# mmigas/LiverRenderer

Hardware: AMD Instinct MI355X
Metric: Msamples/s (higher is better)
Workload: dtype f32; 1 GPU; C3 Liver-SingleMesh volpath 1920x1080 512 spp max_depth 12 (homogeneous medium, isotropic phase, envmap); width=1920, height=1080, spp=512, parallelism=1 GPU

## Files before the change

### liverrenderer_amd/csrc/film.h

```cpp

template <typename FP> DEV float estrin10(float x, FP c) {
    float x2 = x * x, x4 = x2 * x2, x8 = x4 * x4;
    float a0 = fma_(x, c[1], c[0]), a1 = fma_(x, c[3], c[2]), a2 = fma_(x, c[5], c[4]), a3 = fma_(x, c[7], c[6]), a4 = fma_(x, c[9], c[8]);
    float b0 = fma_(x2, a1, a0), b1 = fma_(x2, a3, a2);
    float c0 = fma_(x4, b1, b0);
    return fma_(x8, a4, c0);
}
DEV float rfilter_eval(FilmRef F, float x) {
    if (F.rfilter == LRT_RFILTER_GAUSSIAN) return fmax_(estrin10(sqr(x), F.rf_coeff), 0.f);
    if (F.rfilter == LRT_RFILTER_TENT) return fmax_(0.f, 1.f - __builtin_fabsf(x * F.rf_inv_radius));
    return (x >= -0.5f && x < 0.5f) ? 1.f : 0.f;
}

DEV size_t film_pixel_index(FilmRef F, int px, int py) {
    return (size_t) (py - F.crop_offset_y) * F.width + (px - F.crop_offset_x);
}

struct FilmFootprint {
    int pix, piy; float relx, rely;
    DEV uint32_t key() const { return (uint32_t) (piy + 0x4000) << 16 | (uint32_t) (pix + 0x4000); }
};
DEV FilmFootprint film_footprint(FilmRef F, int px, int py, float jx, float jy) {
    const float spx = (float) px + jx, spy = (float) py + jy;
    FilmFootprint f;
    f.pix = (int) __builtin_floorf(spx) - F.fn; f.piy = (int) __builtin_floorf(spy) - F.fn;
    f.relx = (float) f.pix + .5f - spx; f.rely = (float) f.piy + .5f - spy;
    return f;
}

DEV void finish_path(SceneRef sc, RpRef rp, float *__restrict__ film, float *__restrict__ sample_out,
                     uint64_t sample_base, uint32_t lane, V3 L, bool valid) {
    if (rp.integrator == LRT_INTEGRATOR_PATH && !valid) L = V3(0.f);
    if (sample_out) {
        const uint64_t j = lane_local_index(rp, lane);
        float4 *o = reinterpret_cast<float4 *>(sample_out) + (j - sample_base);
        *o = make_float4(L.x, L.y, L.z, valid ? 1.f : 0.f);
        return;
    }
    FilmRef F = sc.film;
    int px, py; lane_to_pixel(sc, rp, lane, &px, &py);
    const int C = F.channels;
    const float alpha = valid ? 1.f : 0.f;
    auto splat = [&](float *p, float w) {
        atomicAdd(p + 0, L.x * w); atomicAdd(p + 1, L.y * w); atomicAdd(p + 2, L.z * w);
        if (F.has_alpha) { atomicAdd(p + 3, alpha * w); atomicAdd(p + 4, 1.f * w); } else atomicAdd(p + 3, 1.f * w);
    };
    if (F.rfilter == LRT_RFILTER_BOX) {
        int x = px - F.crop_offset_x, y = py - F.crop_offset_y;
        float *p = film + ((size_t) y * F.width + x) * C;
        atomicAdd(p + 0, L.x); atomicAdd(p + 1, L.y); atomicAdd(p + 2, L.z);
        if (F.has_alpha) { atomicAdd(p + 3, alpha); atomicAdd(p + 4, 1.f); } else atomicAdd(p + 3, 1.f);
        return;
    }
    float jx, jy; lane_jitter(rp, lane, lane_local_index(rp, lane), jx, jy);
    const FilmFootprint fp = film_footprint(F, px, py, jx, jy);
    int count = F.fcount;
    for (int ys = 0; ys < count; ++ys) {
        int y = fp.piy - F.crop_offset_y + ys;
        float wy = rfilter_eval(F, fp.rely + (float) ys);
        if (y < 0 || y >= F.height || (wy == 0.f && finite3(L))) continue;
        for (int xs = 0; xs < count; ++xs) {
            int x = fp.pix - F.crop_offset_x + xs;
            if (x < 0 || x >= F.width) continue;
            float w = wy * rfilter_eval(F, fp.relx + (float) xs);
            if (w == 0.f && finite3(L)) continue;
            splat(film + ((size_t) y * F.width + x) * C, w);
        }
    }
}

struct FilmRun { uint32_t pixel; bool head, tail; };
DEV FilmRun film_run(FilmRef F, bool have, int px, int py) {
    FilmRun r;
    r.pixel = have ? (uint32_t) film_pixel_index(F, px, py) : 0xffffffffu;
    const uint32_t prev = wave_prev(r.pixel, 0xfffffffeu), next = wave_next(r.pixel, 0xfffffffeu);
    r.head = r.pixel != prev || !have; r.tail = have && r.pixel != next;
    return r;
}

DEV void finish_paths_wave(SceneRef sc, RpRef rp, float *__restrict__ film, float *__restrict__ sample_out,
                           uint64_t sample_base, bool finishing, uint32_t lane, V3 L, bool valid) {
    FilmRef F = sc.film;
    if (sample_out || F.rfilter != LRT_RFILTER_BOX) {
        if (finishing) finish_path(sc, rp, film, sample_out, sample_base, lane, L, valid);
        return;
    }
    if (rp.integrator == LRT_INTEGRATOR_PATH && !valid) L = V3(0.f);
    uint32_t pixel = 0xffffffffu;
    if (finishing) { int px, py; lane_to_pixel(sc, rp, lane, &px, &py); pixel = (uint32_t) (py - F.crop_offset_y) * (uint32_t) F.width + (uint32_t) (px - F.crop_offset_x); }
    if (__ballot(finishing) == 0ull) return;
    const uint32_t prev = wave_prev(pixel, 0xfffffffeu), next = wave_next(pixel, 0xfffffffeu);
    float v[5] = { finishing ? L.x : 0.f, finishing ? L.y : 0.f, finishing ? L.z : 0.f, finishing ? 1.f : 0.f, (finishing && valid) ? 1.f : 0.f };
    wave_segmented_sums(v, pixel != prev || !finishing);
    if (finishing && pixel != next) {
        float *p = film + (size_t) pixel * F.channels;
        atomicAdd(p + 0, v[0]); atomicAdd(p + 1, v[1]); atomicAdd(p + 2, v[2]);
        if (F.has_alpha) { atomicAdd(p + 3, v[4]); atomicAdd(p + 4, v[3]); } else atomicAdd(p + 3, v[3]);
    }
}

template <int NC, int WI, typename Live, typename Flush>
DEV void film_walk(FilmRef F, bool have, const FilmFootprint &fp, const float (&v)[NC], Live live, Flush flush) {
    const uint32_t me = threadIdx.x & 63u, key = fp.key();
    const int count = F.fcount, n_cells = count * count;
    unsigned long long todo = __ballot(have);
    while (todo) {
        const int leader = __ffsll((long long) todo) - 1;
        const bool mine = have && key == (uint32_t) __shfl((int) key, leader);
        const int gx = __shfl(fp.pix, leader), gy = __shfl(fp.piy, leader);
        float t[NC];
#pragma unroll
        for (int k = 0; k < NC; ++k) t[k] = 0.f;
        for (int ys = 0, ci = 0; ys < count; ++ys) {
            const float wy = mine ? rfilter_eval(F, fp.rely + (float) ys) : 0.f;
            for (int xs = 0; xs < count; ++xs, ++ci) {
                const float w = mine ? wy * rfilter_eval(F, fp.relx + (float) xs) : 0.f;
                const bool keep = (int) me == (ci & 63);
#pragma unroll
                for (int k = 0; k < NC; ++k) {
                    if (!live(k)) continue;
                    const float s = wave_sum(mine ? v[k] * w : 0.f);
                    if (keep) t[k] = s;
                }
                if ((ci & 63) != 63 && ci != n_cells - 1) continue;
                const int cell = (ci & ~63) + (int) me;
                bool add = false;
#pragma unroll
                for (int k = 0; k < NC; ++k) add = add || ((WI < 0 || k == WI) ? t[k] != 0.f : t[k] != t[k]);
                if (cell <= ci && add) {
                    const int cy = cell / count, cx = cell - cy * count;
                    const int x = gx - F.crop_offset_x + cx, y = gy - F.crop_offset_y + cy;
                    if (x >= 0 && x < F.width && y >= 0 && y < F.height) flush(x, y, t);
                }
#pragma unroll
                for (int k = 0; k < NC; ++k) t[k] = 0.f;
            }
        }
        todo &= ~__ballot(mine);
    }
}
```

### liverrenderer_amd/csrc/kernels.h

```cpp
#pragma once
#include "dshade.h"
#include "record.h"

namespace lrt {

#ifndef LRT_STAMP_KIND
#define LRT_STAMP_KIND 0
#endif
struct StampClock {
    unsigned long long *acc; unsigned long long t; bool on;
    DEV void start(unsigned long long *a, bool enable) { acc = a; on = enable; t = on ? __builtin_amdgcn_s_memtime() : 0ull; }
    DEV void at(int k) { if (on) { const unsigned long long now = __builtin_amdgcn_s_memtime(); if ((threadIdx.x & 63u) == 0) atomicAdd(&acc[k], now - t); t = now; } }
};

template <bool LD>
DEV uint64_t lane_rng_inc(RpRef rp, uint32_t lane) {
    if (LD) {
        const uint32_t pixel = (rp.log2_spp != 0xffffffffu) ? (lane >> rp.log2_spp) : (lane / rp.spp);
        uint32_t v0, v1; tea32(rp.base_seed, rp.spp * pixel + rp.seed, &v0, &v1);
        return (uint64_t) v0 | ((uint64_t) (rp.pass_index * rp.spp + (lane - pixel * rp.spp)) << 32);
    }
    uint32_t v0, v1; tea32(rp.seed_value, lane, &v0, &v1);
    return ((uint64_t) v1 << 1) | 1u;
}
template <bool LD>
DEV SamplerT<LD> lane_rng_fresh(RpRef rp, uint32_t lane) {
    SamplerT<LD> r; r.ld_count = rp.ld_count;
    if (LD) { r.state = 0; r.inc = lane_rng_inc<LD>(rp, lane); r.ld_prepare(); return r; }
    uint32_t v0, v1; tea32(rp.seed_value, lane, &v0, &v1);
    r.seed(v0, v1); return r;
}
template <bool LD>
DEV SamplerT<LD> lane_rng_resume(RpRef rp, uint32_t lane, uint64_t state) {
    SamplerT<LD> r; r.ld_count = rp.ld_count; r.state = state; r.inc = lane_rng_inc<LD>(rp, lane); r.ld_prepare(); return r;
}
template <bool LD>
DEV SamplerT<LD> lane_rng_resume_word(RpRef rp, uint32_t lane, uint64_t state, uint32_t word) {
    SamplerT<LD> r; r.ld_count = rp.ld_count; r.state = state;
    if (LD) {
        const uint32_t pixel = (rp.log2_spp != 0xffffffffu) ? (lane >> rp.log2_spp) : (lane / rp.spp);
        r.inc = (uint64_t) word | ((uint64_t) (rp.pass_index * rp.spp + (lane - pixel * rp.spp)) << 32);
    } else r.inc = ((uint64_t) word << 1) | 1u;
    r.ld_prepare(); return r;
}
template <bool LD> DEV uint32_t lane_rng_word(const SamplerT<LD> &r) { return LD ? (uint32_t) r.inc : (uint32_t) (r.inc >> 1); }
DEV uint64_t lane_local_index(RpRef rp, uint32_t lane) {
    if (!rp.pixel_slot) return lane;
    const uint32_t pixel = (rp.log2_spp != 0xffffffffu) ? (lane >> rp.log2_spp) : (lane / rp.spp);
    return (uint64_t) rp.pixel_slot[pixel] * rp.spp + (lane - pixel * rp.spp);
}
DEV uint32_t slot_to_lane(RpRef rp, const uint32_t *__restrict__ pixel_list, uint64_t j) {
    if (!pixel_list) return (uint32_t) j;
    const uint32_t pj = (rp.log2_spp != 0xffffffffu) ? (uint32_t) (j >> rp.log2_spp) : (uint32_t) (j / rp.spp);
    return pixel_list[pj] * rp.spp + (uint32_t) (j - (uint64_t) pj * rp.spp);
}
template <bool LD>
DEV SamplerT<LD> lane_rng_pass_start(RpRef rp, uint32_t lane, uint64_t j) {
    SamplerT<LD> r = lane_rng_fresh<LD>(rp, lane);
    if (!LD && rp.pass_index > 0) r.state = rp.pass_in[j];
    return r;
}
DEV void lane_jitter(RpRef rp, uint32_t lane, uint64_t j, float &jx, float &jy) {
    if (rp.ld_count) { SamplerT<true> r = lane_rng_pass_start<true>(rp, lane, j); r.next2(jx, jy); }
    else { SamplerT<false> r = lane_rng_pass_start<false>(rp, lane, j); r.next2(jx, jy); }
}

DEV void lane_to_pixel(SceneRef sc, RpRef rp, uint32_t lane, int *px, int *py) {
    uint32_t idx = (rp.log2_spp != 0xffffffffu) ? (lane >> rp.log2_spp) : (lane / rp.spp);
    uint32_t W = (uint32_t) sc.film.width;
    uint32_t y = idx / W, x = idx - y * W;
    *px = (int) x + sc.film.crop_offset_x; *py = (int) y + sc.film.crop_offset_y;
}

DEV Ray camera_ray(SceneRef sc, float ax, float ay) {
    const LRT_CONST float *m = sc.cam.s2c;
    V3 p(ax + sc.cam.ppo_x, ay + sc.cam.ppo_y, 0.f);
    float r[4];
#pragma unroll
    for (int i = 0; i < 4; ++i) r[i] = fma_(m[4 * i + 2], p.z, fma_(m[4 * i + 1], p.y, fma_(m[4 * i + 0], p.x, m[4 * i + 3])));
    V3 near_p(r[0] / r[3], r[1] / r[3], r[2] / r[3]);
    V3 d = normalize(near_p);
    Ray ray;
    ray.o = V3(sc.cam.to_world[3], sc.cam.to_world[7], sc.cam.to_world[11]);
    ray.d = xform_vec12(sc.cam.to_world, d);
    float inv_z = rcp(d.z), near_t = sc.cam.near_clip * inv_z, far_t = sc.cam.far_clip * inv_z;
    ray.o = ray.o + ray.d * near_t;
    ray.maxt = far_t - near_t;
    return ray;
}

template <bool LD, bool ENTRY = false>
DEV PathState generate_camera_path(SceneRef sc, RpRef rp, const uint32_t *__restrict__ pixel_list, uint64_t j, uint32_t *entry = nullptr) {
    uint32_t lane;
    if (pixel_list) { uint32_t pj = (rp.log2_spp != 0xffffffffu) ? (uint32_t) (j >> rp.log2_spp) : (uint32_t) (j / rp.spp); lane = pixel_list[pj] * rp.spp + (uint32_t) (j - (uint64_t) pj * rp.spp); }
    else lane = (uint32_t) j;
    if (ENTRY && sc.primary_enabled) *entry = sc.primary_tab[(rp.log2_spp != 0xffffffffu) ? (lane >> rp.log2_spp) : (lane / rp.spp)];
    SamplerT<LD> rng = lane_rng_pass_start<LD>(rp, lane, j);
    int px, py; lane_to_pixel(sc, rp, lane, &px, &py);
    float jx, jy; rng.next2(jx, jy);
    float spx = (float) px + jx, spy = (float) py + jy;
    Ray ray = camera_ray(sc, fma_(spx, sc.film.scale_x, sc.film.offset_x), fma_(spy, sc.film.scale_y, sc.film.offset_y));
    PathState s;
    s.o = ray.o; s.d = ray.d; s.maxt = ray.maxt; s.eta = 1.f; s.tp = V3(1.f); s.res = V3(0.f); s.lp = V3(0.f); s.last_pdf = 1.f; s.lane = lane;
    s.tdepth = 0.f; s.si_t = kInf; s.ff_t = u2f(0x7fc00000u); s.bio_dist = u2f(0x7fc00000u); s.bio_hep = false; s.hit = make_float4(0.f, 0.f, 0.f, 0.f);
    for (int a = 0; a < 2; ++a) for (int i = 0; i < 3; ++i) for (int j = 0; j < 3; ++j) s.W[a][i][j] = 1.f;
    bool env_visible = !rp.hide_emitters && sc.env.type >= 0;
    uint32_t flags = env_visible ? PF_VALID : 0u;
    if (rp.integrator == LRT_INTEGRATOR_PATH) flags |= PF_SPECULAR;
    else {
        if (!rp.hide_emitters) flags |= PF_SPECULAR;
        uint32_t channel = min((uint32_t) (rng.next() * 3.f), 2u);
        flags |= channel << PF_CHANNEL_SHIFT;
        flags |= (uint32_t) (sc.cam.medium + 1) << PF_MEDIUM_SHIFT;
        if (rp.integrator == LRT_INTEGRATOR_BIOVOLPATH06) flags |= PF_BIO_EMIT | PF_BIO_FULL;
    }
    s.flags = flags; s.rng_state = rng.state; s.rng_word = lane_rng_word<LD>(rng);
    return s;
}

#include "film.h"

template <bool HET, typename SMP, typename TR, typename CNT>
DEV V3 volpath_sample_emitter(SceneRef sc, SMP &rng, V3 ref_p, V3 ref_n, bool ref_is_surface, uint32_t ref_shape, V3 ref_geo_n,
                              int medium, uint32_t channel, DirSample *ds_out, const TR &tr, CNT &n_shadow) {
    V3 transmittance(1.f);
    float sx, sy; rng.next2(sx, sy);
    DirSample ds; V3 emitter_val = sample_emitter_direction<TR::kExt>(sc, ref_p, sx, sy, &ds);
    *ds_out = ds;
    if (ds.pdf == 0.f) return V3(0.f);
    Ray ray = spawn_ray_to(ref_p, ref_n, ds.p);
    float max_dist = ray.maxt;
    if (ref_is_surface) { const DShape sd = tab(sc.shapes, ref_shape, sc.one_shape); if (is_medium_transition(sd)) medium = target_medium(sd, ray.d, ref_geo_n); }
    float total_dist = 0.f;
    SI si; si.valid = false; si.t = 0.f; si.shape = 0; si.p = V3(0.f); si.n = V3(0.f);
    bool needs_intersection = true, active = true;
    while (active) {
        float remaining_dist = max_dist - total_dist;
        ray.maxt = remaining_dist;
        if (!(remaining_dist > 0.f)) { rng.skip(1); break; }
        bool escaped_medium = false, active_medium = medium >= 0, active_surface = !active_medium;
        if (!active_medium) rng.skip(1);
        if (active_medium) {
            const DMedium M = tab(sc.media, medium);
            const bool het = HET && M.het;
            MI mei = het ? het_sample_interaction(M, tab(sc.het, medium), ray, rng.next()) : medium_sample_interaction(M, ray, rng.next(), channel);
            if (mei.valid() && !het) ray.maxt = fmin_(mei.t, remaining_dist);
            if (needs_intersection) {
                bool elide = mei.valid() && !sc.has_null_bsdf && !het;
                if (!elide) { n_shadow++; Hit h = tr.closest(ray); si = tr.surface(sc, ray, h); }
                else { si.valid = false; si.t = kInf; }
            }
            if (si.t < mei.t) mei.t = kInf;
            needs_intersection = false;
            bool spectral = M.has_spectral_extinction;
            if (spectral) {
                float t = fmin_(remaining_dist, fmin_(mei.t, si.t)) - mei.mint;
                V3 tr = exp_neg(t, mei.combined);
                V3 ffp = (si.t < mei.t || mei.t > remaining_dist) ? tr : tr * mei.combined;
                float tr_pdf = idx3(ffp, channel);
                transmittance = transmittance * ((tr_pdf > 0.f) ? div_uniform(tr, tr_pdf) : V3(0.f));
            }
            if ((mei.t > remaining_dist) && mei.valid()) total_dist = ds.dist;
            if (mei.t > remaining_dist) mei.t = kInf;
            escaped_medium = !mei.valid();
            active_medium = mei.valid();
            if (active_medium) {
                total_dist += mei.t;
                ray.o = mei.p;
                si.t = si.t - mei.t;
                if (spectral) transmittance = transmittance * mei.sigma_n;
                else transmittance = transmittance * (mei.sigma_n / mei.combined);
            }
        }
        bool intersect = active_surface && needs_intersection;
        if (intersect) { n_shadow++; Hit h = tr.closest(ray); si = tr.surface(sc, ray, h); needs_intersection = false; }
        active_surface = active_surface || escaped_medium;
        if (active_surface) total_dist += si.t;
        active_surface = active_surface && si.valid && !active_medium;
        if (active_surface) {
            transmittance = transmittance * bsdf_null_transmission(sc, tab(sc.shapes, si.shape, sc.one_shape).bsdf);
            ray = spawn_ray(si.p, si.n, ray.d);
        }
        ray.maxt = remaining_dist;
        needs_intersection = needs_intersection || active_surface;
        active = (active_medium || active_surface) && any_nonzero(transmittance);
        if (active_surface) { const DShape sd = tab(sc.shapes, si.shape, sc.one_shape); if (is_medium_transition(sd)) medium = target_medium(sd, ray.d, si.n); }
    }
    return transmittance * emitter_val;
}

struct WaveCount {
    unsigned long long *c;
    DEV void operator++(int) {
        const unsigned long long m = __ballot(true);
        if ((threadIdx.x & 63u) == (uint32_t) (__ffsll((long long) m) - 1)) atomicAdd(c, (unsigned long long) __popcll(m));
    }
};

template <bool HET, bool CLOSED = false, typename SMP, typename TR, typename CNT>
DEV bool volpath_iteration(SceneRef sc, RpRef rp, PathState &s, SMP &rng, const TR &tr, CNT &n_shadow, CNT &n_extra, bool fresh = false, StampClock *clk = nullptr,
                           unsigned long long *guard = nullptr, uint32_t entry = 0u) {
    constexpr bool PRE = !HET;
    uint32_t depth = s.flags & PF_DEPTH_MASK;
    bool proven_empty = (s.flags & PF_NOHIT) != 0;
    float ff_t = s.ff_t;
    const bool needs_intersection = !(HET && (s.flags & PF_HAVE_SI));
    bool act_null_scatter = false;
    Hit hkeep; hkeep.t = s.hit.x; hkeep.u = s.hit.y; hkeep.v = s.hit.z; hkeep.prim = f2u(s.hit.w);
    if (PRE) { hkeep.t = kInf; hkeep.u = hkeep.v = 0.f; hkeep.prim = 0xffffffffu; }
    int medium = (int) ((s.flags & PF_MEDIUM_MASK) >> PF_MEDIUM_SHIFT) - 1;
    const uint32_t channel = (s.flags >> PF_CHANNEL_SHIFT) & 3u;
    bool specular_chain = (s.flags & PF_SPECULAR) != 0, valid_ray = (s.flags & PF_VALID) != 0;
    const uint32_t max_depth = (uint32_t) rp.max_depth;
    V3 throughput = s.tp, result = CLOSED ? V3(0.f) : s.res;
    bool broken = false;
    float eta = s.eta;
    Ray ray; ray.o = s.o; ray.d = s.d; ray.maxt = s.maxt;
    auto commit = [&]() {
        s.tp = throughput; s.res = result; s.eta = eta; s.o = ray.o; s.d = ray.d; s.maxt = ray.maxt;
        s.flags = (depth & PF_DEPTH_MASK) | ((uint32_t) (medium + 1) << PF_MEDIUM_SHIFT) | (channel << PF_CHANNEL_SHIFT) |
                  (specular_chain ? PF_SPECULAR : 0u) | (valid_ray ? PF_VALID : 0u);
    };
    auto termination_stage = [&]() -> bool {
        bool a = any_nonzero(throughput);
        const float q = fmin_(max3(throughput) * sqr(eta), .95f);
        const bool perform_rr = depth > (uint32_t) rp.rr_depth;
        if (a) { const float u = rng.next(); a = (u < q) || !perform_rr; }
        if (perform_rr) throughput = throughput * rcp(q);
        return a && depth < max_depth;
    };
    uint32_t nohit = 0;
    float cache_t = u2f(0x7fc00000u);
    float cone_free = 0.f;
    auto free_flight_stage = [&]() {
        if (medium < 0) return;
        const DMedium M = tab(sc.media, medium);
        cache_t = medium_sampled_t(M, rng.next(), channel);
        if (sc.grid.enabled) {
            const MI m2 = medium_interaction_at(M, ray, cache_t);
            if (m2.valid() && (CLOSED ? segment_free_of_surfaces_from(sc.grid, ray.o, ray.d, m2.t, cone_free) : segment_free_of_surfaces(sc.grid, ray.o, ray.d, m2.t))) nohit = PF_NOHIT;
        }
    };
    bool active = true;
    if (!PRE) active = termination_stage();
    else if (fresh) { active = termination_stage(); if (active && !CLOSED) { free_flight_stage(); ff_t = cache_t; proven_empty = nohit != 0; nohit = 0; cache_t = u2f(0x7fc00000u); } }
    if (!active) { commit(); return false; }

    bool active_medium = medium >= 0, active_surface = !active_medium;
    bool act_medium_scatter = false, escaped_medium = false;
    MI mei; mei.t = kInf;
    SI si; si.valid = false; si.t = kInf;
    if (!active_medium) rng.skip(2);
    if (active_medium) {
        const DMedium M = tab(sc.media, medium);
        const bool het = HET && M.het;
        if (PRE) mei = medium_interaction_at(M, ray, ff_t);
        else { const float sample = rng.next(); mei = het ? het_sample_interaction(M, tab(sc.het, medium), ray, sample) : medium_sample_interaction(M, ray, sample, channel); }
        if (mei.valid() && !het) ray.maxt = mei.t;
        if (!needs_intersection) si = surface_of(tr, sc, ray, hkeep);
// ... 119 lines not shown
    }
    active_surface = active_surface && si.valid;
    if (!active_surface) rng.skip(3);
    if (active_surface) {
        uint4 cone_rows = make_uint4(0u, 0u, 0u, 0u);
        if (CLOSED && sc.cone_enabled) cone_rows = *reinterpret_cast<const uint4 *>(sc.cone_tab + 2u * (size_t) si.prim);
        const DShape sd = tab(sc.shapes, si.shape, sc.one_shape);
        int b = sd.bsdf;
        int flags = tab(sc.bsdfs, b, sc.one_shape).flags;
        bool active_e = !CLOSED && (flags & F_SMOOTH) && (depth + 1 < max_depth);
        if (!active_e) rng.skip(1);
        if (active_e) {
            DirSample ds;
            V3 emitted = volpath_sample_emitter<HET>(sc, rng, si.p, si.n, true, si.shape, si.n, medium, channel, &ds, tr, n_shadow);
            V3 wo = si.sh.to_local(ds.d);
            V3 bsdf_val = bsdf_eval<TR::kExt>(sc, b, si, wo);
            float bpdf = bsdf_pdf<TR::kExt>(sc, b, si, wo);
            V3 c = throughput * bsdf_val * mis_weight(ds.pdf, ds.delta ? 0.f : bpdf) * emitted;
            result = result + c;
        }
        float s1 = rng.next(), s2x, s2y; rng.next2(s2x, s2y);
        const BSDFSample bs = bsdf_sample<CLOSED, TR::kExt>(sc, b, si, s1, s2x, s2y);
        throughput = throughput * bs.weight;
        eta *= bs.eta;
        ray = spawn_ray(si.p, si.n, si.sh.to_world(bs.wo));
        bool non_null = !(bs.type & F_NULL);
        if (non_null) { depth += 1; s.lp = si.p; s.last_pdf = bs.pdf; valid_ray = true; }
        specular_chain = specular_chain || (non_null && (bs.type & F_DELTA));
        specular_chain = specular_chain && !(bs.type & F_SMOOTH);
        if (is_medium_transition(sd)) medium = target_medium(sd, ray.d, si.n);
        if (CLOSED && sc.cone_enabled) cone_free = cone_free_length(cone_rows, ray.d, si.n);
    }
    active = active && (active_surface || active_medium);
    if (clk) clk->at(3);
    if (PRE) {
        if (active) { if (!termination_stage()) { active = false; n_extra++; } else free_flight_stage(); }
        if (clk) clk->at(4);
    } else if (active) {
        SMP pk = rng;
        bool a2 = any_nonzero(throughput);
        float q2 = fmin_(max3(throughput) * sqr(eta), .95f);
        if (a2) { float u = pk.next(); a2 = (u < q2) || !(depth > (uint32_t) rp.rr_depth); }
        a2 = a2 && depth < max_depth;
        if (!a2) { active = false; n_extra++; rng = pk; }
        else if (medium >= 0 && sc.grid.enabled && !(HET && act_null_scatter)) {
            const DMedium M = tab(sc.media, medium);
            if (!(HET && M.het)) {
                const float t2 = medium_sampled_t(M, pk.next(), channel);
                const MI m2 = medium_interaction_at(M, ray, t2);
                if (m2.valid() && segment_free_of_surfaces(sc.grid, ray.o, ray.d, m2.t)) nohit = PF_NOHIT;
            }
        }
    }
    commit();
    s.flags |= nohit; s.ff_t = cache_t;
#ifndef LRT_CLOSED_NO_GUARD
    if (CLOSED && (broken || (active && !(result.x == 0.f && result.y == 0.f && result.z == 0.f)))) atomicAdd(guard, 1ull);
#endif
    if (HET && act_null_scatter && active) { s.flags |= PF_HAVE_SI; s.hit = make_float4(hkeep.t, hkeep.u, hkeep.v, u2f(hkeep.prim)); }
    return active;
}

template <typename SMP, typename TR>
DEV bool path_iteration(SceneRef sc, RpRef rp, PathState &s, SMP &rng, const TR &tr, uint32_t &n_shadow) {
    uint32_t depth = s.flags & PF_DEPTH_MASK;
    bool prev_bsdf_delta = (s.flags & PF_SPECULAR) != 0, valid_ray = (s.flags & PF_VALID) != 0;
    const uint32_t max_depth = (uint32_t) rp.max_depth;
    V3 throughput = s.tp, result = s.res;
    float eta = s.eta;
    Ray ray; ray.o = s.o; ray.d = s.d; ray.maxt = s.maxt;
    auto commit = [&]() {
        s.tp = throughput; s.res = result; s.eta = eta; s.o = ray.o; s.d = ray.d; s.maxt = ray.maxt;
        s.flags = (depth & PF_DEPTH_MASK) | (prev_bsdf_delta ? PF_SPECULAR : 0u) | (valid_ray ? PF_VALID : 0u);
    };
    if (max_depth == 0) { commit(); return false; }
    Hit pi = tr.closest(ray);
    if (rp.hide_emitters && depth == 0) {
        bool skip = hit_on_emitter(tr, sc, pi);
        if (skip) {
            SI s0 = surface_of(tr, sc, ray, pi);
            Ray r2 = spawn_ray(s0.p, s0.n, ray.d);
            bool a = true; Hit h; h.prim = 0xffffffffu; h.t = kInf; h.u = h.v = 0.f;
            while (a) {
                h = tr.closest(r2);
                a = hit_on_emitter(tr, sc, h);
                if (a) { SI s2 = surface_of(tr, sc, r2, h); r2 = spawn_ray(s2.p, s2.n, r2.d); }
            }
            pi = h; ray = r2;
        }
    }
    SI si = surface_of(tr, sc, ray, pi);
    int emitter = si_emitter(sc, si);
    if (emitter >= 0) {
        float em_pdf = 0.f;
        if (!prev_bsdf_delta) em_pdf = pdf_emitter_direction<TR::kExt>(sc, s.lp, si, emitter);
        float mis_bsdf = mis_weight(s.last_pdf, em_pdf);
        V3 em = (s.last_pdf > 0.f) ? emitter_eval(sc, emitter, si) : V3(0.f);
        em = em * mis_bsdf;
        result = V3(fma_(throughput.x, em.x, result.x), fma_(throughput.y, em.y, result.y), fma_(throughput.z, em.z, result.z));
    }
    bool active_next = (depth + 1 < max_depth) && si.valid;
    if (!active_next) {
        float a0, a1; rng.next2(a0, a1); (void) rng.next(); rng.next2(a0, a1); (void) rng.next();
        if (si.valid && !(tab(sc.bsdfs, tab(sc.shapes, si.shape, sc.one_shape).bsdf, sc.one_shape).flags & F_NULL)) valid_ray = true;
        commit(); return false;
    }
    const DShape sd = tab(sc.shapes, si.shape, sc.one_shape);
    int b = sd.bsdf;
    bool active_em = (tab(sc.bsdfs, b, sc.one_shape).flags & F_SMOOTH) != 0;
    DirSample ds; ds.pdf = 0.f; ds.delta = false; ds.d = V3(0.f);
    V3 em_weight(0.f), wo(0.f);
    float sx, sy; rng.next2(sx, sy);
    if (active_em) {
        em_weight = sample_emitter_direction<TR::kExt>(sc, si.p, sx, sy, &ds);
        if (ds.pdf != 0.f) {
            Ray sr = spawn_ray_to(si.p, si.n, ds.p);
            n_shadow++;
            Hit h = tr.any(sr);
            if (h.prim != 0xffffffffu) { em_weight = V3(0.f); ds.pdf = 0.f; }
        }
        active_em = ds.pdf != 0.f;
        wo = si.sh.to_local(ds.d);
    }
    float s1 = rng.next(), s2x, s2y; rng.next2(s2x, s2y);
    V3 bsdf_val = bsdf_eval<TR::kExt>(sc, b, si, wo);
    float bpdf = bsdf_pdf<TR::kExt>(sc, b, si, wo);
    const BSDFSample bs = bsdf_sample<false, TR::kExt>(sc, b, si, s1, s2x, s2y);
    const V3 bsdf_weight = bs.weight;
    if (active_em) {
        float mis_em = ds.delta ? 1.f : mis_weight(ds.pdf, bpdf);
        V3 c = bsdf_val * em_weight * mis_em;
        result = V3(fma_(throughput.x, c.x, result.x), fma_(throughput.y, c.y, result.y), fma_(throughput.z, c.z, result.z));
    }
    ray = spawn_ray(si.p, si.n, si.sh.to_world(bs.wo));
    throughput = throughput * bsdf_weight;
    eta *= bs.eta;
    valid_ray = valid_ray || !(bs.type & F_NULL);
    s.lp = si.p; s.last_pdf = bs.pdf; prev_bsdf_delta = (bs.type & F_DELTA) != 0;
    depth += 1;
    float tmax = max3(throughput);
    float rr_prob = fmin_(tmax * sqr(eta), .95f);
    bool rr_active = depth >= (uint32_t) rp.rr_depth, rr_continue = rng.next() < rr_prob;
    if (rr_active) throughput = throughput * rcp(rr_prob);
    bool active = active_next && (!rr_active || rr_continue) && (tmax != 0.f);
    commit();
    return active;
}

}
#include "kernels_bio.h"
#include "kernels_mis.h"
namespace lrt {

template <RecordLayout LAYOUT = RecordLayout::Wide, bool READLANE = true, bool COMPACT = false, bool LONGQ = false>
DEV void retire_and_compact_wave(SceneRef sc, RpRef rp, bool had_path, bool alive, const PathState &s,
                                 float *__restrict__ film, float *__restrict__ sample_out, uint64_t sample_base,
                                 const LRT_CONST DPathStreams &qout, size_t pool, uint32_t P, uint32_t *s_out , StampClock *clk = nullptr) {
    const uint32_t lane_in_wave = threadIdx.x & 63u;
    const int region = !(s.flags & PF_MEDIUM_MASK) ? 2 : ((s.flags & PF_NOHIT) ? 0 : ((LONGQ && (s.flags & PF_LONG_QUERY)) ? 3 : 1));
    const unsigned long long m0 = __ballot(alive && region == 0), m1 = __ballot(alive && region == 1), m2 = __ballot(alive && region == 2);
    const unsigned long long m3 = LONGQ ? __ballot(alive && region == 3) : 0ull;
    uint32_t base = 0;
    if (lane_in_wave < (LONGQ ? 4u : 3u)) {
        const uint32_t c = (uint32_t) __popcll(lane_in_wave == 0 ? m0 : (lane_in_wave == 1 ? m1 : ((!LONGQ || lane_in_wave == 2) ? m2 : m3)));
        if (c) base = atomicAdd(&s_out[lane_in_wave], c);
    }
    uint32_t b;
    if (READLANE) {
        const uint32_t b0 = (uint32_t) __builtin_amdgcn_readlane((int) base, 0), b1 = (uint32_t) __builtin_amdgcn_readlane((int) base, 1), b2 = (uint32_t) __builtin_amdgcn_readlane((int) base, 2);
        b = region == 0 ? b0 : (region == 1 ? b1 : b2);
        if (LONGQ) { const uint32_t b3 = (uint32_t) __builtin_amdgcn_readlane((int) base, 3); if (region == 3) b = b3; }
    } else b = __shfl(base, region);
    if (clk) clk->at(5);
    if (alive) {
        const unsigned long long mine = region == 0 ? m0 : (region == 1 ? m1 : ((!LONGQ || region == 2) ? m2 : m3));
        const uint32_t slot = b + (uint32_t) __popcll(mine & ((1ull << lane_in_wave) - 1ull));
        store_state<LAYOUT, COMPACT>(qout, pool + (region == 0 ? slot : (region == 1 ? P + slot : ((!LONGQ || region == 2) ? 2u * P - 1u - slot : P - 1u - slot))), s);
    }
    if (clk) clk->at(6);
    if (rp.pass_out && had_path && !alive) rp.pass_out[lane_local_index(rp, s.lane)] = s.rng_state;
    finish_paths_wave(sc, rp, film, sample_out, sample_base, had_path && !alive, s.lane, s.res, (s.flags & PF_VALID) != 0);
}

template <int INTEGRATOR, int BLOCK, bool LDS_BVH, bool LD, bool COMPACT = false, bool EXT = false>
__global__ void __launch_bounds__(BLOCK, BLOCK == 512 ? 2 : (BLOCK == 768 ? 3 : 4))
k_render(ScenePtr scp, LaunchPtr lp) {
    SceneRef sc = *scp;
    const LRT_CONST DLaunch &A = *lp;
    RpRef rp = A.rp;
    const LRT_CONST DLdsInfo &li = A.li;
    const uint32_t P = A.P;
    extern __shared__ __align__(16) unsigned char smem[];
    __shared__ uint32_t s_in[4], s_out[4], s_ticket, s_fresh;
    __shared__ unsigned long long s_fresh_base, s_prof[8];
#ifdef LRT_STAMP
    __shared__ unsigned long long s_stamp[16];
    if (threadIdx.x < 16) s_stamp[threadIdx.x] = 0;
#endif
    const uint32_t tid = threadIdx.x, lane_in_wave = tid & 63u;
    constexpr bool READLANE = INTEGRATOR != LRT_INTEGRATOR_PATH && INTEGRATOR != LRT_INTEGRATOR_BIOVOLPATH06;
    constexpr bool LONGQ = INTEGRATOR == LRT_INTEGRATOR_BIOVOLPATH;
    constexpr bool CLOSED = INTEGRATOR == LRT_INTEGRATOR_VOLPATH_CLOSED;
    constexpr RecordLayout LAYOUT = record_layout(INTEGRATOR);
    if (tid < 8) s_prof[tid] = 0;
    const unsigned long long t_wg_start = (rp.profile & 1u) ? wall_clock64() : 0ull;
    unsigned long long t_loop_start = 0ull, t_barrier = 0ull;
    LdsScene L{};
    if (LDS_BVH) {
        const uint4 *src = li.blob; uint4 *dst = reinterpret_cast<uint4 *>(smem);
        for (uint32_t k = tid; k < li.blob_bytes / 16u; k += BLOCK) dst[k] = src[k];
        L.nodes = reinterpret_cast<const float4 *>(smem + li.nodes_off); L.verts = reinterpret_cast<const float4 *>(smem + li.verts_off);
        L.tris = reinterpret_cast<const uint2 *>(smem + li.tris_off);
        L.n_faces = sc.n_faces; L.root_is_leaf = (uint32_t) sc.root_is_leaf; L.root_first = sc.root_leaf_first; L.root_count = sc.root_leaf_count;
    }
    const LdsTracer<BLOCK> tr_lds_tri{ L, reinterpret_cast<uint16_t *>(smem + li.stack_off) + tid };
    const GlobalTracer tr_glb_tri{ sc, reinterpret_cast<int *>(smem) + tid };
    const ExtTracer<LdsTracer<BLOCK>> tr_lds_ext{ tr_lds_tri, sc };
    const ExtTracer<GlobalTracer> tr_glb_ext{ tr_glb_tri, sc };
    const auto &tr_lds = pick<EXT>(tr_lds_tri, tr_lds_ext);
    const auto &tr_glb = pick<EXT>(tr_glb_tri, tr_glb_ext);
    const size_t pool = (size_t) blockIdx.x * 2u * P;
    uint32_t parity = 0;
    if (tid == 0) { s_in[0] = s_in[1] = s_in[2] = 0; if (LONGQ) s_in[3] = 0; }
    bool lanes_left = true;
    constexpr bool VP_LDS_COUNT = INTEGRATOR == LRT_INTEGRATOR_VOLPATH || CLOSED;
    __shared__ unsigned long long s_cnt[2];
    if (VP_LDS_COUNT && tid < 2) s_cnt[tid] = 0;
    WaveCount wc_shadow{ &s_cnt[0] }, wc_extra{ &s_cnt[1] };
    uint32_t n_shadow = 0, n_extra = 0, n_trips = 0, n_loaded = 0;
    uint32_t n_proven = 0;
    uint32_t n_primary = 0;
    if (rp.profile & 1u) t_loop_start = wall_clock64();
    for (;;) {
        if (tid == 0) {
            const uint32_t want = P - (s_in[0] + s_in[1] + s_in[2] + (LONGQ ? s_in[3] : 0u));
            uint32_t got = 0; unsigned long long base = 0;
            if (want && lanes_left) {
                base = atomicAdd(&A.cnt->next_lane, (unsigned long long) want);
                if (base < rp.n_lanes) got = (uint32_t) (rp.n_lanes - base < (unsigned long long) want ? rp.n_lanes - base : (unsigned long long) want);
                lanes_left = base + want < rp.n_lanes;
            }
            s_fresh = got; s_fresh_base = base; s_ticket = 0; s_out[0] = s_out[1] = s_out[2] = 0; if (LONGQ) s_out[3] = 0;
        }
        __syncthreads();
        const uint32_t n_a = s_in[0], n_c = s_in[1], n_b = s_in[2], n_l = LONGQ ? s_in[3] : 0u, fresh = s_fresh;
        const unsigned long long fresh_base = s_fresh_base;
        if (n_a + n_c + n_b + n_l + fresh == 0) break;
        const uint32_t ta = (n_a + 63u) >> 6, tc = (n_c + 63u) >> 6, tb = (n_b + 63u) >> 6, tf = (fresh + 63u) >> 6;
        const uint32_t tcl = tc + (LONGQ ? (n_l + 63u) >> 6 : 0u);
        const uint32_t n_tiles = ta + tcl + tb + tf;
        for (;;) {
            uint32_t t = 0;
            if (lane_in_wave == 0) t = atomicAdd(&s_ticket, 1u);
            t = (uint32_t) __builtin_amdgcn_readfirstlane((int) t);
            if (t >= n_tiles) break;
            const unsigned long long t_begin = (rp.profile & 1u) ? wall_clock64() : 0ull;
#ifdef LRT_STAMP
            StampClock clk; clk.start(s_stamp, LRT_STAMP_KIND == 0 ? t < ta : (LRT_STAMP_KIND == 1 ? (t >= ta && t < ta + tcl) : (LRT_STAMP_KIND == 2 ? (t >= ta + tcl && t < ta + tcl + tb) : t >= ta + tcl + tb)));
#endif
            bool had_path = false, alive = false;
            PathState s; s.flags = 0; s.lane = 0; s.res = V3(0.f);
            uint32_t entry = 0u;
            if (t < ta + tcl + tb) {
                uint32_t i;
                if (t < ta) { i = (t << 6) + lane_in_wave; had_path = i < n_a; }
                else if (t < ta + tc) { i = ((t - ta) << 6) + lane_in_wave; had_path = i < n_c; i += P; }
                else if (LONGQ && t < ta + tcl) { i = ((t - ta - tc) << 6) + lane_in_wave; had_path = i < n_l; i = P - 1u - i; }
                else { i = ((t - ta - tcl) << 6) + lane_in_wave; had_path = i < n_b; i = 2u * P - 1u - i; }
                if (had_path) { load_state<LAYOUT, COMPACT>(parity ? A.q1 : A.q0, pool + i, s); if (!VP_LDS_COUNT) n_loaded += 1; }
            } else {
                const uint32_t i = ((t - ta - tcl - tb) << 6) + lane_in_wave;
                had_path = i < fresh;
                if (had_path) s = generate_camera_path<LD, CLOSED>(sc, rp, A.pixel_list, A.lane_begin + fresh_base + i, &entry);
                if (CLOSED && sc.primary_enabled) n_primary += (uint32_t) __popcll(__ballot(entry != 0u));
            }
            if (VP_LDS_COUNT) {
                const uint32_t n_had = (uint32_t) __popcll(__ballot(had_path));
                n_trips += n_had;
                if (t < ta + tcl + tb) n_loaded += n_had;
                if (CLOSED && t < ta) n_proven += n_had;
            }
#ifdef LRT_STAMP
            clk.at(0);
#endif
            if (had_path) {
                SamplerT<LD> rng = COMPACT ? lane_rng_resume_word<LD>(rp, s.lane, s.rng_state, s.rng_word) : lane_rng_resume<LD>(rp, s.lane, s.rng_state);
#ifdef LRT_STAMP
                clk.at(1);
#endif
                if (INTEGRATOR == LRT_INTEGRATOR_PATH) alive = LDS_BVH ? path_iteration(sc, rp, s, rng, tr_lds, n_shadow) : path_iteration(sc, rp, s, rng, tr_glb, n_shadow);
                else if (INTEGRATOR == LRT_INTEGRATOR_BIOVOLPATH) { const bool fresh_tile = t >= ta + tcl + tb; alive = LDS_BVH ? biovolpath_iteration(sc, rp, s, rng, tr_lds, n_shadow, n_extra, fresh_tile) : biovolpath_iteration(sc, rp, s, rng, tr_glb, n_shadow, n_extra, fresh_tile); }
                else if (INTEGRATOR == LRT_INTEGRATOR_BIOVOLPATH06) alive = LDS_BVH ? biovolpath06_iteration(sc, rp, s, rng, tr_lds) : biovolpath06_iteration(sc, rp, s, rng, tr_glb);
                else if (INTEGRATOR == LRT_INTEGRATOR_VOLPATHMIS) alive = LDS_BVH ? volpathmis_iteration<true>(sc, rp, s, rng, tr_lds, n_shadow) : volpathmis_iteration<true>(sc, rp, s, rng, tr_glb, n_shadow);
                else if (INTEGRATOR == LRT_INTEGRATOR_VOLPATHMIS_PLAIN) alive = LDS_BVH ? volpathmis_iteration<false>(sc, rp, s, rng, tr_lds, n_shadow) : volpathmis_iteration<false>(sc, rp, s, rng, tr_glb, n_shadow);
                else if (INTEGRATOR == LRT_INTEGRATOR_VOLPATH_HET) alive = LDS_BVH ? volpath_iteration<true>(sc, rp, s, rng, tr_lds, n_shadow, n_extra) : volpath_iteration<true>(sc, rp, s, rng, tr_glb, n_shadow, n_extra);
                else {
                    const bool fresh_tile = t >= ta + tcl + tb;
#ifdef LRT_STAMP
                    StampClock *const pclk = &clk;
#else
                    StampClock *const pclk = nullptr;
#endif
                    unsigned long long *const guard = CLOSED ? &A.cnt->n_closed_guard : nullptr;
                    alive = LDS_BVH ? volpath_iteration<false, CLOSED>(sc, rp, s, rng, tr_lds, wc_shadow, wc_extra, fresh_tile, pclk, guard, entry) : volpath_iteration<false, CLOSED>(sc, rp, s, rng, tr_glb, wc_shadow, wc_extra, fresh_tile, pclk, guard, entry);
                }
                s.rng_state = rng.state;
                if (!VP_LDS_COUNT) n_trips += 1;
            }
#ifdef LRT_STAMP
            retire_and_compact_wave<LAYOUT, READLANE, COMPACT, LONGQ>(sc, rp, had_path, alive, s, A.film, A.sample_out, A.sample_base, parity ? A.q0 : A.q1, pool, P, s_out, &clk);
            clk.at(7);
            if (clk.on && lane_in_wave == 0) atomicAdd(&s_stamp[15], 1ull);
#else
            retire_and_compact_wave<LAYOUT, READLANE, COMPACT, LONGQ>(sc, rp, had_path, alive, s, A.film, A.sample_out, A.sample_base, parity ? A.q0 : A.q1, pool, P, s_out);
#endif
            if ((rp.profile & 1u) && lane_in_wave == 0) {
                const int region = t < ta ? 0 : (t < ta + tcl ? 1 : (t < ta + tcl + tb ? 2 : 3));
                atomicAdd(&s_prof[region], wall_clock64() - t_begin); atomicAdd(&s_prof[4 + region], 1ull);
            }
        }
        { const unsigned long long tb0 = (rp.profile & 1u) ? wall_clock64() : 0ull;
        __syncthreads();
        if (rp.profile & 1u) t_barrier += wall_clock64() - tb0; }
        if (tid == 0) { s_in[0] = s_out[0]; s_in[1] = s_out[1]; s_in[2] = s_out[2]; if (LONGQ) s_in[3] = s_out[3]; }
        parity ^= 1u;
    }
    if ((rp.profile & 1u) && (tid & 63u) == 0) {
        const unsigned long long t_end = wall_clock64();
        if (tid == 0) { atomicAdd(&A.cnt->prof_wg[0], t_loop_start - t_wg_start); atomicMax(&A.cnt->prof_wg[1], t_end); atomicMax(&A.cnt->prof_wg[2], ~t_wg_start); atomicAdd(&A.cnt->prof_wg[3], t_end - t_wg_start); atomicMax(&A.cnt->prof_wg[5], t_wg_start); }
        atomicAdd(&A.cnt->prof_wg[4], t_barrier);
    }
    if ((rp.profile & 1u) && tid < 8) { if (tid < 4) atomicAdd(&A.cnt->prof_cycles[tid], s_prof[tid]); else atomicAdd(&A.cnt->prof_tiles[tid - 4], s_prof[tid]); }
#ifdef LRT_TRAV_STATS
    if (tid == 0 && blockIdx.x == 0) printf("[trav, so far] closest: node steps %llu (lanes %.1f), leaf steps %llu (lanes %.1f); any-hit: node steps %llu (lanes %.1f), leaf steps %llu (lanes %.1f)\n", g_trav[0], (double) g_trav[1] / g_trav[0], g_trav[2], (double) g_trav[3] / g_trav[2], g_trav[4], (double) g_trav[5] / g_trav[4], g_trav[6], (double) g_trav[7] / g_trav[6]);
#endif
#ifdef LRT_STAMP
    __syncthreads();
    if (tid == 0 && blockIdx.x == 7) printf("[stamp] tiles of kind %d in workgroup 7: %llu; cycles per tile: ticket+load issue %.0f, record wait+TEA %.0f, to the end of the medium interaction / ray query %.0f, scatter + surface %.0f, termination+free flight %.0f, ballots+slots %.0f, stores %.0f, film %.0f\n", LRT_STAMP_KIND, s_stamp[15],
        (double) s_stamp[0] / s_stamp[15], (double) s_stamp[1] / s_stamp[15], (double) s_stamp[2] / s_stamp[15], (double) s_stamp[3] / s_stamp[15], (double) s_stamp[4] / s_stamp[15], (double) s_stamp[5] / s_stamp[15], (double) s_stamp[6] / s_stamp[15], (double) s_stamp[7] / s_stamp[15]);
#endif
    if (!VP_LDS_COUNT) {
        n_trips += n_extra;
        for (int off = 32; off > 0; off >>= 1) {
            n_shadow += __shfl_down(n_shadow, off); n_trips += __shfl_down(n_trips, off); n_loaded += __shfl_down(n_loaded, off);
        }
    }
    if (lane_in_wave == 0) {
        if (!VP_LDS_COUNT && n_shadow) atomicAdd(&A.cnt->n_shadow, (unsigned long long) n_shadow);
        if (n_trips) atomicAdd(&A.cnt->n_iter, (unsigned long long) n_trips);
        if (n_loaded) atomicAdd(&A.cnt->n_records, (unsigned long long) n_loaded);
        if (CLOSED && n_proven) atomicAdd(&A.cnt->n_proven, (unsigned long long) n_proven);
        if (CLOSED && n_primary) atomicAdd(&A.cnt->n_primary_entry, (unsigned long long) n_primary);
    }
    if (VP_LDS_COUNT) {
        __syncthreads();
        if (tid == 0) {
            if (s_cnt[0]) atomicAdd(&A.cnt->n_shadow, s_cnt[0]);
            if (s_cnt[1]) atomicAdd(&A.cnt->n_iter, s_cnt[1]);
        }
    }
}

DEV float point_triangle_dist2(V3 p, V3 a, V3 ab, V3 ac) {
    V3 ap = p - a;
    float d1 = dot(ab, ap), d2 = dot(ac, ap);
    if (d1 <= 0.f && d2 <= 0.f) return dot(ap, ap);
    V3 bp = ap - ab;
    float d3 = dot(ab, bp), d4 = dot(ac, bp);
    if (d3 >= 0.f && d4 <= d3) return dot(bp, bp);
    float vc = d1 * d4 - d3 * d2;
    if (vc <= 0.f && d1 >= 0.f && d3 <= 0.f) { V3 r = ap - ab * (d1 / (d1 - d3)); return dot(r, r); }
    V3 cp = ap - ac;
    float d5 = dot(ab, cp), d6 = dot(ac, cp);
    if (d6 >= 0.f && d5 <= d6) return dot(cp, cp);
    float vb = d5 * d2 - d1 * d6;
    if (vb <= 0.f && d2 >= 0.f && d6 <= 0.f) { V3 r = ap - ac * (d2 / (d2 - d6)); return dot(r, r); }
    float va = d3 * d6 - d5 * d4;
    if (va <= 0.f && (d4 - d3) >= 0.f && (d5 - d6) >= 0.f) { V3 r = bp - (ac - ab) * ((d4 - d3) / ((d4 - d3) + (d5 - d6))); return dot(r, r); }
    float denom = 1.f / (va + vb + vc);
    V3 r = ap - ab * (vb * denom) - ac * (vc * denom);
    return dot(r, r);
}

__global__ void __launch_bounds__(LRT_BLOCK)
k_build_dist_grid(const float4 *__restrict__ tris, uint32_t n_slots, DDistGrid g, uint16_t *__restrict__ out, float abs_margin,
                  const DSphere *__restrict__ spheres, uint32_t n_spheres) {
    const size_t n_cells = (size_t) g.n[0] * g.n[1] * g.n[2];
    const size_t c = (size_t) blockIdx.x * LRT_BLOCK + threadIdx.x;
    if (c >= n_cells) return;
    const int ix = (int) (c % g.n[0]), iy = (int) ((c / g.n[0]) % g.n[1]), iz = (int) (c / ((size_t) g.n[0] * g.n[1]));
    const V3 p(g.lo[0] + ((float) ix + .5f) * g.cell, g.lo[1] + ((float) iy + .5f) * g.cell, g.lo[2] + ((float) iz + .5f) * g.cell);
    float best = kInf;
    for (uint32_t sl = 0; sl < n_slots; ++sl) {
        const float4 a = tris[3 * sl], b = tris[3 * sl + 1], cc = tris[3 * sl + 2];
        float d2 = point_triangle_dist2(p, V3(a.x, a.y, a.z), V3(b.x, b.y, b.z), V3(cc.x, cc.y, cc.z));
        if (!(d2 >= 0.f)) d2 = 0.f;
        best = fmin_(best, d2);
    }
    for (uint32_t k = 0; k < n_spheres; ++k) {
        const DSphere &S = spheres[k];
        const float ds = __builtin_fabsf(norm(p - V3(S.center[0], S.center[1], S.center[2])) - S.radius);
        best = fmin_(best, ds * ds);
    }
    float d = __builtin_sqrtf(best) * .999f - abs_margin;
    d = d > 0.f ? fmin_(d, 60000.f) : 0.f;
    union { uint16_t u; _Float16 h; } cv; cv.h = (_Float16) d;
    if ((float) cv.h > d) cv.u -= 1;
    out[c] = cv.u;
}

template <bool WEIGHTS_ONLY>
__global__ void __launch_bounds__(LRT_BLOCK)
k_splat_lanes(ScenePtr scp, LaunchPtr lp) {
    RpRef rp = lp->rp;
    const float4 *__restrict__ lane_L = lp->L_buf; const uint32_t *__restrict__ pixel_list = lp->pixel_list;
    const uint64_t slot_base = lp->lane_begin, n = lp->n;
    float *__restrict__ film = lp->film;
    SceneRef sc = *scp;
    FilmRef F = sc.film;
    const uint64_t i = (uint64_t) blockIdx.x * LRT_BLOCK + threadIdx.x;
    const uint32_t me = threadIdx.x & 63u;
    const bool have = i < n;
    V3 L(0.f); float alpha = 0.f; FilmFootprint fp{}; uint32_t key = 0xffffffffu;
    if (have) {
        const uint64_t j = slot_base + i;
        const uint32_t lane = slot_to_lane(rp, pixel_list, j);
        if (!WEIGHTS_ONLY) {
            const float4 v = lane_L[i];
            L = V3(v.x, v.y, v.z); alpha = v.w;
            if (rp.integrator == LRT_INTEGRATOR_PATH && alpha == 0.f) L = V3(0.f);
        }
        int px, py; lane_to_pixel(sc, rp, lane, &px, &py);
        float jx, jy; lane_jitter(rp, lane, j, jx, jy);
        fp = film_footprint(F, px, py, jx, jy);
        key = fp.key();
    }
    const float relx = fp.relx, rely = fp.rely; const int pix = fp.pix, piy = fp.piy;
    const int count = F.fcount, C = F.channels;
    unsigned long long todo = __ballot(have);
    while (todo) {
        const int leader = __ffsll((long long) todo) - 1;
        const uint32_t k0 = __shfl(key, leader);
        const bool mine = have && key == k0;
        const int gx = __shfl(pix, leader), gy = __shfl(piy, leader);
        float tr = 0.f, tg = 0.f, tb = 0.f, ta = 0.f, tw = 0.f;
        const int n_cells = count * count;
        for (int ys = 0, ci = 0; ys < count; ++ys) {
            const float wy = mine ? rfilter_eval(F, rely + (float) ys) : 0.f;
            for (int xs = 0; xs < count; ++xs, ++ci) {
                const float w = mine ? wy * rfilter_eval(F, relx + (float) xs) : 0.f;
                float r = mine ? L.x * w : 0.f, g = mine ? L.y * w : 0.f, b = mine ? L.z * w : 0.f, a = alpha * w, ww = w;
                if (!WEIGHTS_ONLY) { r = wave_sum(r); g = wave_sum(g); b = wave_sum(b); if (F.has_alpha) a = wave_sum(a); }
                ww = wave_sum(ww);
                if ((int) me == (ci & 63)) { tr = r; tg = g; tb = b; ta = a; tw = ww; }
                if ((ci & 63) == 63 || ci == n_cells - 1) {
                    const int cell = (ci & ~63) + (int) me;
                    if (cell <= ci && (tw != 0.f || tr != tr || tg != tg || tb != tb)) {
                        const int cy = cell / count, cx = cell - cy * count;
                        const int x = gx - F.crop_offset_x + cx, y = gy - F.crop_offset_y + cy;
                        if (x >= 0 && x < F.width && y >= 0 && y < F.height) {
                            if (WEIGHTS_ONLY) atomicAdd(film + (size_t) y * F.width + x, tw);
                            else {
                                float *p = film + ((size_t) y * F.width + x) * C;
                                atomicAdd(p + 0, tr); atomicAdd(p + 1, tg); atomicAdd(p + 2, tb);
                                if (F.has_alpha) { atomicAdd(p + 3, ta); atomicAdd(p + 4, tw); } else atomicAdd(p + 3, tw);
                            }
                        }
// ... 59 lines not shown
```

Before: 6910 Msamples/s.

## Count film sample weights at path birth and skip splats for unlit paths

In the closed-loop volpath kernel, each box-filtered pixel's sample count (and alpha, when it is known at birth) is now added once per wave run when camera paths are generated. Path retirement then uses a new routine that returns early if no finishing lane carries nonzero radiance and skips the RGB atomics for zero sums. The goal is fewer segmented reductions and film atomics at retirement. The cost is an extra ballot/shuffle pass and atomics at path birth, and correctness now depends on the birth-time count matching the paths that actually finish.

```diff
diff --git a/liverrenderer_amd/csrc/film.h b/liverrenderer_amd/csrc/film.h
--- a/liverrenderer_amd/csrc/film.h
+++ b/liverrenderer_amd/csrc/film.h
@@ -99,6 +99,44 @@
     }
 }
 
+DEV uint32_t lane_film_pixel(RpRef rp, uint32_t lane) { return (rp.log2_spp != 0xffffffffu) ? (lane >> rp.log2_spp) : (lane / rp.spp); }
+
+DEV void count_born_wave(SceneRef sc, RpRef rp, float *__restrict__ film, const float *__restrict__ sample_out, bool born, uint32_t pixel) {
+    FilmRef F = sc.film;
+    if (sample_out || F.rfilter != LRT_RFILTER_BOX) return;
+    const uint32_t prev = wave_prev(pixel, 0xfffffffeu), next = wave_next(pixel, 0xfffffffeu);
+    const unsigned long long heads = __ballot(pixel != prev || !born), members = __ballot(born);
+    if (born && pixel != next) {
+        float *p = film + (size_t) pixel * (uint32_t) F.channels;
+        const float n = (float) film_run_count(heads, members, threadIdx.x & 63u);
+        atomicAdd(p + F.channels - 1, n);
+        if (F.has_alpha && LRT_BORN_VALID(sc, rp)) atomicAdd(p + 3, n);
+    }
+}
+
+DEV void finish_paths_wave_closed(SceneRef sc, RpRef rp, float *__restrict__ film, float *__restrict__ sample_out,
+                                  uint64_t sample_base, bool finishing, uint32_t lane, V3 L, bool valid) {
+    FilmRef F = sc.film;
+    if (sample_out || F.rfilter != LRT_RFILTER_BOX) {
+        if (finishing) finish_path(sc, rp, film, sample_out, sample_base, lane, L, valid);
+        return;
+    }
+    const unsigned long long lit = __ballot(finishing && (L.x != 0.f || L.y != 0.f || L.z != 0.f));
+    const unsigned long long opaque = (F.has_alpha && !LRT_BORN_VALID(sc, rp)) ? __ballot(finishing && valid) : 0ull;
+    if ((lit | opaque) == 0ull) return;
+    const uint32_t pixel = finishing ? lane_film_pixel(rp, lane) : 0xffffffffu;
+    const uint32_t prev = wave_prev(pixel, 0xfffffffeu), next = wave_next(pixel, 0xfffffffeu);
+    const bool head = pixel != prev || !finishing;
+    float v[3] = { finishing ? L.x : 0.f, finishing ? L.y : 0.f, finishing ? L.z : 0.f };
+    if (lit) wave_segmented_sums(v, head);
+    const unsigned long long heads = opaque ? __ballot(head) : 0ull;
+    if (finishing && pixel != next) {
+        float *p = film + (size_t) pixel * (uint32_t) F.channels;
+        if (v[0] != 0.f || v[1] != 0.f || v[2] != 0.f) { atomicAdd(p + 0, v[0]); atomicAdd(p + 1, v[1]); atomicAdd(p + 2, v[2]); }
+        if (opaque) atomicAdd(p + 3, (float) film_run_count(heads, opaque, threadIdx.x & 63u));
+    }
+}
+
 template <int NC, int WI, typename Live, typename Flush>
 DEV void film_walk(FilmRef F, bool have, const FilmFootprint &fp, const float (&v)[NC], Live live, Flush flush) {
     const uint32_t me = threadIdx.x & 63u, key = fp.key();
diff --git a/liverrenderer_amd/csrc/film_runs.h b/liverrenderer_amd/csrc/film_runs.h
--- /dev/null
+++ b/liverrenderer_amd/csrc/film_runs.h
@@ -0,0 +1,23 @@
+#pragma once
+#include <cstdint>
+
+namespace lrt {
+
+constexpr uint64_t film_run_lanes(uint64_t heads, uint32_t i) {
+    const uint64_t upto = ~0ull >> (63u - i);
+    const uint32_t start = 63u - (uint32_t) __builtin_clzll((heads | 1ull) & upto);
+    return upto & (~0ull << start);
+}
+constexpr uint32_t film_popcount(uint64_t m) { return (uint32_t) __builtin_popcount((uint32_t) m) + (uint32_t) __builtin_popcount((uint32_t) (m >> 32)); }
+constexpr uint32_t film_run_count(uint64_t heads, uint64_t members, uint32_t i) {
+    return film_popcount(members & film_run_lanes(heads, i));
+}
+constexpr uint32_t film_run_count_of(uint64_t heads, uint64_t members, uint64_t which, uint32_t i) {
+    return film_popcount(which & members & film_run_lanes(heads, i));
+}
+
+static_assert(film_run_count(0ull, ~0ull, 63u) == 64u && film_run_count(~0ull, ~0ull, 63u) == 1u, "one run of 64 lanes; 64 runs of one");
+static_assert(film_run_count(1ull << 40, ~0ull, 63u) == 24u && film_run_count(1ull << 40, ~0ull, 39u) == 40u, "a run that ends at lane 63; the one before it");
+static_assert(film_run_count_of(1ull << 8, 0xff00ull, 0x5500ull, 15u) == 4u && film_run_count_of(1ull << 8, 0xf0ffull, 0xffffull, 15u) == 4u, "a third mask; a member mask with holes");
+
+}
diff --git a/liverrenderer_amd/csrc/kernels.h b/liverrenderer_amd/csrc/kernels.h
--- a/liverrenderer_amd/csrc/kernels.h
+++ b/liverrenderer_amd/csrc/kernels.h
@@ -1,6 +1,7 @@
 #pragma once
 #include "dshade.h"
 #include "record.h"
+#include "film_runs.h"
 
 namespace lrt {
 
@@ -89,12 +90,17 @@
     return ray;
 }
 
+#define LRT_BORN_VALID(sc, rp) (!(rp).hide_emitters && (sc).env.type >= 0)
+
 template <bool LD, bool ENTRY = false>
-DEV PathState generate_camera_path(SceneRef sc, RpRef rp, const uint32_t *__restrict__ pixel_list, uint64_t j, uint32_t *entry = nullptr) {
+DEV PathState generate_camera_path(SceneRef sc, RpRef rp, const uint32_t *__restrict__ pixel_list, uint64_t j, uint32_t *entry = nullptr, uint32_t *film_pixel = nullptr) {
     uint32_t lane;
     if (pixel_list) { uint32_t pj = (rp.log2_spp != 0xffffffffu) ? (uint32_t) (j >> rp.log2_spp) : (uint32_t) (j / rp.spp); lane = pixel_list[pj] * rp.spp + (uint32_t) (j - (uint64_t) pj * rp.spp); }
     else lane = (uint32_t) j;
-    if (ENTRY && sc.primary_enabled) *entry = sc.primary_tab[(rp.log2_spp != 0xffffffffu) ? (lane >> rp.log2_spp) : (lane / rp.spp)];
+    if (ENTRY) {
+        *film_pixel = (rp.log2_spp != 0xffffffffu) ? (lane >> rp.log2_spp) : (lane / rp.spp);
+        if (sc.primary_enabled) *entry = sc.primary_tab[*film_pixel];
+    }
     SamplerT<LD> rng = lane_rng_pass_start<LD>(rp, lane, j);
     int px, py; lane_to_pixel(sc, rp, lane, &px, &py);
     float jx, jy; rng.next2(jx, jy);
@@ -104,7 +110,7 @@
     s.o = ray.o; s.d = ray.d; s.maxt = ray.maxt; s.eta = 1.f; s.tp = V3(1.f); s.res = V3(0.f); s.lp = V3(0.f); s.last_pdf = 1.f; s.lane = lane;
     s.tdepth = 0.f; s.si_t = kInf; s.ff_t = u2f(0x7fc00000u); s.bio_dist = u2f(0x7fc00000u); s.bio_hep = false; s.hit = make_float4(0.f, 0.f, 0.f, 0.f);
     for (int a = 0; a < 2; ++a) for (int i = 0; i < 3; ++i) for (int j = 0; j < 3; ++j) s.W[a][i][j] = 1.f;
-    bool env_visible = !rp.hide_emitters && sc.env.type >= 0;
+    bool env_visible = LRT_BORN_VALID(sc, rp);
     uint32_t flags = env_visible ? PF_VALID : 0u;
     if (rp.integrator == LRT_INTEGRATOR_PATH) flags |= PF_SPECULAR;
     else {
@@ -530,7 +536,7 @@
 #include "kernels_mis.h"
 namespace lrt {
 
-template <RecordLayout LAYOUT = RecordLayout::Wide, bool READLANE = true, bool COMPACT = false, bool LONGQ = false>
+template <RecordLayout LAYOUT = RecordLayout::Wide, bool READLANE = true, bool COMPACT = false, bool LONGQ = false, bool COUNTED = false>
 DEV void retire_and_compact_wave(SceneRef sc, RpRef rp, bool had_path, bool alive, const PathState &s,
                                  float *__restrict__ film, float *__restrict__ sample_out, uint64_t sample_base,
                                  const LRT_CONST DPathStreams &qout, size_t pool, uint32_t P, uint32_t *s_out , StampClock *clk = nullptr) {
@@ -557,7 +563,8 @@
     }
     if (clk) clk->at(6);
     if (rp.pass_out && had_path && !alive) rp.pass_out[lane_local_index(rp, s.lane)] = s.rng_state;
-    finish_paths_wave(sc, rp, film, sample_out, sample_base, had_path && !alive, s.lane, s.res, (s.flags & PF_VALID) != 0);
+    if (COUNTED) finish_paths_wave_closed(sc, rp, film, sample_out, sample_base, had_path && !alive, s.lane, s.res, (s.flags & PF_VALID) != 0);
+    else finish_paths_wave(sc, rp, film, sample_out, sample_base, had_path && !alive, s.lane, s.res, (s.flags & PF_VALID) != 0);
 }
 
 template <int INTEGRATOR, int BLOCK, bool LDS_BVH, bool LD, bool COMPACT = false, bool EXT = false>
@@ -649,8 +656,10 @@
             } else {
                 const uint32_t i = ((t - ta - tcl - tb) << 6) + lane_in_wave;
                 had_path = i < fresh;
-                if (had_path) s = generate_camera_path<LD, CLOSED>(sc, rp, A.pixel_list, A.lane_begin + fresh_base + i, &entry);
+                uint32_t film_pixel = 0xffffffffu;
+                if (had_path) s = generate_camera_path<LD, CLOSED>(sc, rp, A.pixel_list, A.lane_begin + fresh_base + i, &entry, &film_pixel);
                 if (CLOSED && sc.primary_enabled) n_primary += (uint32_t) __popcll(__ballot(entry != 0u));
+                if (CLOSED) count_born_wave(sc, rp, A.film, A.sample_out, had_path, film_pixel);
             }
             if (VP_LDS_COUNT) {
                 const uint32_t n_had = (uint32_t) __popcll(__ballot(had_path));
@@ -686,11 +695,11 @@
                 if (!VP_LDS_COUNT) n_trips += 1;
             }
 #ifdef LRT_STAMP
-            retire_and_compact_wave<LAYOUT, READLANE, COMPACT, LONGQ>(sc, rp, had_path, alive, s, A.film, A.sample_out, A.sample_base, parity ? A.q0 : A.q1, pool, P, s_out, &clk);
+            retire_and_compact_wave<LAYOUT, READLANE, COMPACT, LONGQ, CLOSED>(sc, rp, had_path, alive, s, A.film, A.sample_out, A.sample_base, parity ? A.q0 : A.q1, pool, P, s_out, &clk);
             clk.at(7);
             if (clk.on && lane_in_wave == 0) atomicAdd(&s_stamp[15], 1ull);
 #else
-            retire_and_compact_wave<LAYOUT, READLANE, COMPACT, LONGQ>(sc, rp, had_path, alive, s, A.film, A.sample_out, A.sample_base, parity ? A.q0 : A.q1, pool, P, s_out);
+            retire_and_compact_wave<LAYOUT, READLANE, COMPACT, LONGQ, CLOSED>(sc, rp, had_path, alive, s, A.film, A.sample_out, A.sample_base, parity ? A.q0 : A.q1, pool, P, s_out);
 #endif
             if ((rp.profile & 1u) && lane_in_wave == 0) {
                 const int region = t < ta ? 0 : (t < ta + tcl ? 1 : (t < ta + tcl + tb ? 2 : 3));
```

After: 7351 Msamples/s, median of 6. 6.4% higher.
